# aleju/cat-generator

Measured on AMD Instinct MI355X. Metric: images/sec per G+D step, G32up-c 32x32 RGB bs=128 per GPU, higher is better.
Workload: dtype f32

## Files before the change

cat-generator_amd/csrc/common.h:

```cpp
#pragma once
#include <hip/hip_runtime.h>
#include <algorithm>
#include <stdint.h>
#include <stdio.h>
#include <string.h>
#include "../../include/catgan.h"

namespace cg {

char* err_buf();
int fail(const char* fmt, ...);

inline hipStream_t S(void* s) { return reinterpret_cast<hipStream_t>(s); }

#define CG_HIP(call)                                                              \
    do {                                                                          \
        hipError_t e__ = (call);                                                  \
        if (e__ != hipSuccess)                                                    \
            return cg::fail("%s:%d %s -> %s", __FILE__, __LINE__, #call,          \
                            hipGetErrorString(e__));                              \
    } while (0)

#define CG_LAUNCH_CHECK()                                                         \
    do {                                                                          \
        hipError_t e__ = hipGetLastError();                                       \
        if (e__ != hipSuccess)                                                    \
            return cg::fail("%s:%d kernel launch -> %s", __FILE__, __LINE__,      \
                            hipGetErrorString(e__));                              \
    } while (0)

#define CG_REQUIRE(cond, ...)                                                     \
    do {                                                                          \
        if (!(cond)) return cg::fail(__VA_ARGS__);                                \
    } while (0)

constexpr int kNumCU = 256;

#ifndef CG_TIMING_PROBE
#define CG_TIMING_PROBE 0
#endif
#define CG_PROBE_HALF(fam, T) (((CG_TIMING_PROBE) & (fam)) ? ((T) + 1) / 2 : (T))
constexpr int kEwWgsPerCU = 4, kColReduceWgsPerCU = 1;

enum Opt {
    OPT_SKINNY, OPT_GEMM_BK32, OPT_WINO_BK, OPT_NN_TILE, OPT_TN_TILE, OPT_NN_SPLITS, OPT_TN_SPLITS,
    OPT_XCD_SWIZZLE, OPT_NN_GLDS, OPT_TN_GLDS, OPT_WINO_GLDS, OPT_PAD_SKIP, OPT_WINO3, OPT_WINO_DGRAD_FUSE, OPT_WINO_DGRAD_FUSE_LAUNCHES,
    OPT_WINO3_LAUNCHES, OPT_PACK_WIDE, OPT_SAMPLER_ATOMIC_LAUNCHES, OPT_COUNT
};
long opt(Opt o);
void opt_count(Opt o);

static inline int cdiv(long a, long b) { return (int)((a + b - 1) / b); }

constexpr size_t kColScratchBytes = 8u << 20;
void* col_scratch(hipStream_t stream);
hipStream_t queue_stream(hipStream_t ref, int cls, int slot);
int queue_class(hipStream_t ref, hipStream_t s);

constexpr int MAXG = 4;
constexpr int kMaxStridedGroups = 36;
template <typename T>
__device__ __forceinline__ T sel4(int i, T a, T b, T c, T d) { return i == 0 ? a : (i == 1 ? b : (i == 2 ? c : d)); }
__device__ __forceinline__ float4 ld4(const float* p) { return *reinterpret_cast<const float4*>(p); }
__device__ __forceinline__ float f4c(const float4& v, int i) { return i == 0 ? v.x : (i == 1 ? v.y : (i == 2 ? v.z : v.w)); }
template <typename T>
static inline void set4(T& p0, T& p1, T& p2, T& p3, const T* src, int n) {
    T* const dst[MAXG] = {&p0, &p1, &p2, &p3};
    for (int i = 0; i < MAXG; ++i) *dst[i] = (src && i < n) ? src[i] : nullptr;
}
__device__ __host__ __forceinline__ int phase_map(int a, int d, int pad) { return ((a + d - pad) >> 1) - ((a - pad) >> 1); }
static inline int phase_kp(int k, int pad) { return phase_map(0, k - 1, pad) + 1; }

struct WgradParts {
    const float* part;
    const float* bias_part;
    float* const* gw;
    float* const* gb;
    long gws;
    int ngroups, S, Cin, Cout, kH, kW, pad, ups;
    float scale;
};
int wgrad_finish(hipStream_t st, const WgradParts& w, bool defer);
void wgrad_discard_all();

constexpr int kSkinnyWgradBlocks = 512;
bool skinny_ok(int ngroups, int Cin, int Cout, int kH, int kW, int padH, int padW, int ups);
size_t skinny_wgrad_ws_bytes(int Cin, int Cout);
void skinny_valu_forward(hipStream_t st, const float* x, const float* w, const float* bias, float* y, int N, int H, int W, int Cin, int Cout);
void skinny_valu_wgrad(hipStream_t st, const float* x, const float* dy, float* part, float* bias_part, int N, int H, int W, int Cin, int Cout,
                       int blocks, long ppb);
bool skinny_mfma_ok(int Cin, int Cout, int H, int W);
int skinny_mfma_forward(hipStream_t st, const float* x, const float* w, const float* bias, float* y, int N, int H, int W, int Cin, int Cout);
int skinny_mfma_wgrad(hipStream_t st, const float* x, const float* dy, float* part, float* bias_part, int N, int H, int W, int Cin, int Cout,
                      int max_blocks);

bool head_wgrad_ok(int N, int T, int C, int Co);
int head_wgrad(hipStream_t st, const float* x, const float* dy, float* gw, float* gb, int N, int T, int C, int Co, float scale);
constexpr int kWino3UOffset = 9 * 64 * 64, kWino3UFloats = 16 * 64 * 64;
static inline bool wino3_layer(int Cout, int Cin, int kH, int kW) { return Cout == 64 && Cin == 64 && kH == 3 && kW == 3; }
bool wino3_geom_ok(int ngroups, int N, int H, int W, int Cin, int Cout, int kH, int kW, int padH, int padW, int ups);
int wino3_note_pack(hipStream_t st, int n, const float* const* w, float* const* wf, float* const* wb, const int* Cout, const int* Cin,
                    const int* kH, const int* kW, const int* wb_map);
int wino3_forward(hipStream_t st, int ngroups, const float* const* x, const float* const* wpk, const float* const* bias, float* const* y,
                  int N, int H, int W);

static inline int ew_grid(long n, int per_block = 256) {
    long b = (n + per_block - 1) / per_block;
    if (b < 1) b = 1;
    const long cap = (long)kNumCU * kEwWgsPerCU;
    if (b > cap) b = cap;
    return (int)b;
}

static inline bool al16(const void* p) { return ((uintptr_t)p & 15) == 0; }
template <class... P>
static inline bool vec_ok(long n, const P*... p) { return n % 4 == 0 && (al16(p) && ...); }
// ... 247 lines not shown
```

cat-generator_amd/csrc/gemm.hip:

```cpp
#include "common.h"
#include <stdlib.h>
#include <algorithm>
#include <type_traits>

using cg::f4c;
using cg::kMaxStridedGroups;
using cg::ld4;
using cg::MAXG;
using cg::phase_kp;
using cg::sel4;
using cg::set4;

namespace {

typedef float f32x16 __attribute__((ext_vector_type(16)));
typedef unsigned int u32x4 __attribute__((ext_vector_type(4)));

constexpr int BK = 16;
constexpr unsigned OOB = 0x80000000u;
#ifdef CG_TRACE
__device__ unsigned long long* g_trace;
#define CG_STAMP(slot)                                                                                                  \
    do {                                                                                                                \
        if (threadIdx.x == 0 && g_trace) {                                                                              \
// ... 1735 lines not shown
}

int cg_conv2d_dgrad_ups2(void* stream, const float* dy, const float* wb_ph, float* dx_lo, int N, int Hp, int Wp, int Cin,
                         int Cout, int k, int pad, void* ws, size_t ws_bytes) {
    CG_REQUIRE(dy && wb_ph && dx_lo, "cg_conv2d_dgrad_ups2: null pointer");
    Geom g;
    if (check_dims(N, Hp, Wp, Cin, Cout, k, k, pad, pad, 1)) return 1;
    if (geom_phase_dgrad(g, N, Hp, Wp, Cin, Cout, k, pad)) return 1;
    return run_nn(cg::S(stream), g, 1, &dy, &wb_ph, nullptr, &dx_lo, ws, ws_bytes, "cg_conv2d_dgrad_ups2");
}

static size_t wgrad_ws_bytes_groups(int ngroups, int maxg, int N, int Hp, int Wp, int Cin, int Cout, int kH, int kW, int padH, int padW, int ups) {
    Geom g;
    if (ngroups < 1 || ngroups > maxg || conv_geom(g, N, Hp, Wp, Cin, Cout, kH, kW, padH, padW, ups)) return 0;
    const size_t reg = tn_ws_bytes(g, plan_tn(g, ngroups), ngroups);
    return cg::skinny_ok(ngroups, Cin, Cout, kH, kW, padH, padW, ups) ? std::max(reg, cg::skinny_wgrad_ws_bytes(Cin, Cout)) : reg;
}
size_t cg_conv2d_wgrad_workspace_bytes_grouped(int ngroups, int N, int Hp, int Wp, int Cin, int Cout, int kH, int kW,
                                               int padH, int padW, int ups) {
    return wgrad_ws_bytes_groups(ngroups, MAXG, N, Hp, Wp, Cin, Cout, kH, kW, padH, padW, ups);
}
size_t cg_conv2d_wgrad_workspace_bytes_strided(int ngroups, int N, int Hp, int Wp, int Cin, int Cout, int kH, int kW,
                                               int padH, int padW, int ups) {
    return wgrad_ws_bytes_groups(ngroups, kMaxStridedGroups, N, Hp, Wp, Cin, Cout, kH, kW, padH, padW, ups);
}
size_t cg_conv2d_wgrad_workspace_bytes(int N, int Hp, int Wp, int Cin, int Cout, int kH, int kW, int padH, int padW,
                                       int ups) {
    return cg_conv2d_wgrad_workspace_bytes_grouped(1, N, Hp, Wp, Cin, Cout, kH, kW, padH, padW, ups);
}

namespace {
int wgrad_impl(void* stream, int ngroups, const float* const* x, const float* const* dy, float* const* gw, float* const* gb, int N,
               int Hp, int Wp, int Cin, int Cout, int kH, int kW, int padH, int padW, int ups, float scale, void* ws, size_t ws_bytes,
               bool defer, long xgs = 0, long dgs = 0, long gws = 0, bool gemm_only = false);
}

int cg_conv2d_wgrad_grouped(void* stream, int ngroups, const float* const* x, const float* const* dy, float* const* gw,
                            float* const* gb, int N, int Hp, int Wp, int Cin, int Cout, int kH, int kW, int padH, int padW,
                            int ups, float scale, void* ws, size_t ws_bytes) {
    return wgrad_impl(stream, ngroups, x, dy, gw, gb, N, Hp, Wp, Cin, Cout, kH, kW, padH, padW, ups, scale, ws, ws_bytes, false);
}

int cg_conv2d_wgrad_grouped_deferred(void* stream, int ngroups, const float* const* x, const float* const* dy, float* const* gw,
                                     float* const* gb, int N, int Hp, int Wp, int Cin, int Cout, int kH, int kW, int padH, int padW,
                                     int ups, float scale, void* ws, size_t ws_bytes) {
    return wgrad_impl(stream, ngroups, x, dy, gw, gb, N, Hp, Wp, Cin, Cout, kH, kW, padH, padW, ups, scale, ws, ws_bytes, true);
}

int cg_conv2d_wgrad_strided(void* stream, int ngroups, const float* x, long x_stride, const float* dy, long dy_stride, float* gw,
                            long gw_stride, int N, int Hp, int Wp, int Cin, int Cout, int kH, int kW, int padH, int padW, int ups,
                            float scale, void* ws, size_t ws_bytes) {
    CG_REQUIRE(x && dy && gw && x_stride > 0 && dy_stride > 0 && gw_stride > 0, "cg_conv2d_wgrad_strided: bad arguments");
    CG_REQUIRE(ngroups >= 1 && ngroups <= kMaxStridedGroups, "cg_conv2d_wgrad_strided: 1..%d groups per launch", kMaxStridedGroups);
    return wgrad_impl(stream, ngroups, &x, &dy, &gw, nullptr, N, Hp, Wp, Cin, Cout, kH, kW, padH, padW, ups, scale, ws, ws_bytes, false,
                      x_stride, dy_stride, gw_stride);
}

int cg_conv2d_wgrad_gemm(void* stream, const float* x, const float* dy, int N, int Hp, int Wp, int Cin, int Cout, int kH, int kW, int padH,
                         int padW, int ups, void* ws, size_t ws_bytes) {
    CG_REQUIRE(x && dy && ws, "cg_conv2d_wgrad_gemm: null pointer");
    CG_REQUIRE(!cg::skinny_ok(1, Cin, Cout, kH, kW, padH, padW, ups), "cg_conv2d_wgrad_gemm: this geometry runs the skinny kernel, not the GEMM");
    float* gw = (float*)ws;
    return wgrad_impl(stream, 1, &x, &dy, &gw, nullptr, N, Hp, Wp, Cin, Cout, kH, kW, padH, padW, ups, 1.f, ws, ws_bytes, false, 0, 0, 0, true);
}

namespace {
void launch_tn_tile(const TNArgs& a, const TileCfg& tc, bool tng, dim3 grid, hipStream_t st, bool veca, bool vecb) {
    if (tng) {
        if (tc.bm == 128 && tc.bn == 128) launch_tng<128, 128, 2, 2>(a, grid, st);
        else if (tc.bm == 64 && tc.bn == 128) launch_tng<64, 128, 2, 2>(a, grid, st);
        else if (tc.bm == 128 && tc.bn == 64) launch_tng<128, 64, 2, 2>(a, grid, st);
        else if (tc.bm == 64 && tc.bn == 64) launch_tng<64, 64, 2, 2>(a, grid, st);
        else launch_tng<128, 32, 4, 1>(a, grid, st);
    }
    else if (tc.bm == 128 && tc.bn == 128) launch_tn<128, 128, 2, 2>(a, grid, st, veca, vecb);
    else if (tc.bm == 64 && tc.bn == 128) launch_tn<64, 128, 2, 2>(a, grid, st, veca, vecb);
    else if (tc.bm == 128 && tc.bn == 64) launch_tn<128, 64, 2, 2>(a, grid, st, veca, vecb);
    else if (tc.bm == 64 && tc.bn == 64) launch_tn<64, 64, 2, 2>(a, grid, st, veca, vecb);
    else launch_tn<128, 32, 4, 1>(a, grid, st, veca, vecb);
}

int wgrad_impl(void* stream, int ngroups, const float* const* x, const float* const* dy, float* const* gw, float* const* gb, int N,
               int Hp, int Wp, int Cin, int Cout, int kH, int kW, int padH, int padW, int ups, float scale, void* ws, size_t ws_bytes,
               bool defer, long xgs, long dgs, long gws_, bool gemm_only) {
    CG_REQUIRE(x && dy && gw, "cg_conv2d_wgrad: null pointer");
    const bool strided = xgs != 0;
    CG_REQUIRE(ngroups >= 1 && ngroups <= (strided ? kMaxStridedGroups : MAXG), "cg_conv2d_wgrad: 1..%d groups per launch", strided ? kMaxStridedGroups : MAXG);
    CG_REQUIRE(!strided || (!gb && !defer), "cg_conv2d_wgrad: strided groups carry no bias gradient and are not deferred");
    TNArgs a;
    memset(&a, 0, sizeof(a));
    if (conv_geom(a.g, N, Hp, Wp, Cin, Cout, kH, kW, padH, padW, ups)) return 1;
    const Geom& g = a.g;
    if (!strided && cg::skinny_ok(ngroups, Cin, Cout, kH, kW, padH, padW, ups) && x[0] && dy[0] && gw[0] && (uintptr_t)x[0] % 16 == 0 && ws &&
        ws_bytes >= cg::skinny_wgrad_ws_bytes(Cin, Cout) && (long)N * Hp * Wp < 0x7fffffffL) {
        hipStream_t st = cg::S(stream);
        const long npix = (long)N * Hp * Wp;
        const long ppb = (npix + cg::kSkinnyWgradBlocks - 1) / cg::kSkinnyWgradBlocks;
        int blocks = (int)((npix + ppb - 1) / ppb);
        float* part = (float*)ws;
        float* bpart = part + (size_t)cg::kSkinnyWgradBlocks * 9 * Cin * Cout;
        float* gb0 = gb ? gb[0] : nullptr;
        if (cg::opt(cg::OPT_SKINNY) == 1 && cg::skinny_mfma_ok(Cin, Cout, Hp, Wp)) {
            blocks = cg::skinny_mfma_wgrad(st, x[0], dy[0], part, gb0 ? bpart : nullptr, N, Hp, Wp, Cin, Cout, cg::kSkinnyWgradBlocks / 2);
            if (blocks < 0) return 1;
        }
        else cg::skinny_valu_wgrad(st, x[0], dy[0], part, gb0 ? bpart : nullptr, N, Hp, Wp, Cin, Cout, blocks, ppb);
        CG_LAUNCH_CHECK();
        const cg::WgradParts parts{part, gb0 ? bpart : nullptr, gw, gb, 0, 1, blocks, Cin, Cout, 3, 3, 1, 0, scale};
        return cg::wgrad_finish(st, parts, defer);
    }
    if (!strided && !gemm_only && ngroups == 1 && !ups && kH == Hp && kW == Wp && padH == 0 && padW == 0 && cg::opt(cg::OPT_PAD_SKIP) > 0 &&
        cg::opt(cg::OPT_TN_GLDS) && cg::head_wgrad_ok(N, kH * kW, Cin, Cout) && x[0] && dy[0] && gw[0] && (uintptr_t)x[0] % 16 == 0 &&
        (uintptr_t)dy[0] % 16 == 0 && (uintptr_t)gw[0] % 4 == 0)
        return cg::head_wgrad(cg::S(stream), x[0], dy[0], gw[0], gb ? gb[0] : nullptr, N, kH * kW, Cin, Cout, scale) != 0;
    TNPlan p = plan_tn(g, ngroups);
    const size_t need = tn_ws_bytes(g, p, ngroups);
    CG_REQUIRE(ws && ws_bytes >= need, "cg_conv2d_wgrad: workspace too small (%zu < %zu)", ws_bytes, need);
    const int nptr = strided ? 1 : ngroups;
    bool veca = Cin % 4 == 0, vecb = Cout % 4 == 0, any_gb = false;
    for (int i = 0; i < nptr; ++i) {
        CG_REQUIRE(x[i] && dy[i] && gw[i], "cg_conv2d_wgrad: null pointer (group %d)", i);
        veca = veca && ((uintptr_t)x[i] % 16 == 0);
        vecb = vecb && ((uintptr_t)dy[i] % 16 == 0);
        any_gb = any_gb || (gb && gb[i]);
    }
    if (strided) { veca = veca && xgs % 4 == 0; vecb = vecb && dgs % 4 == 0; }
    if (p.pm && !(veca && vecb)) p = plan_tn(g, ngroups, false);
    a.xgs = xgs; a.dgs = dgs;
    set4(a.x0, a.x1, a.x2, a.x3, x, nptr);
    set4(a.d0, a.d1, a.d2, a.d3, dy, nptr);
    a.ngroups = ngroups; a.part = (float*)ws; a.pchunk = p.pchunk;
    a.xcd_swizzle = (int)cg::opt(cg::OPT_XCD_SWIZZLE);
    const int ZP = ngroups * g.nphase;
    const long wplane = (long)g.Ktot * g.Cout;
    a.bias_part = any_gb ? (float*)ws + (size_t)p.splits * ZP * wplane : nullptr;
    hipStream_t st = cg::S(stream);
    dim3 grid(cg::cdiv(g.Ktot, p.tc.bm) * cg::cdiv(g.Cout, p.tc.bn), p.splits, ZP);
    if (p.pm && veca && vecb) a.pm_n = g.M / (g.Hg * g.Wg);
    launch_tn_tile(a, p.tc, a.pm_n || tng_ok(g, p.pchunk, veca, vecb), grid, st, veca, vecb);
    CG_LAUNCH_CHECK();
    if (gemm_only) return 0;
    const cg::WgradParts parts{(const float*)ws, a.bias_part, gw, gb, strided ? gws_ : 0, ngroups, p.splits, Cin, Cout, kH, kW, padH, ups, scale};
    return cg::wgrad_finish(st, parts, defer);
}

}

int cg_conv2d_wgrad(void* stream, const float* x, const float* dy, float* gw, float* gb, int N, int Hp, int Wp, int Cin,
                    int Cout, int kH, int kW, int padH, int padW, int ups, float scale, void* ws, size_t ws_bytes) {
    CG_REQUIRE(x && dy && gw, "cg_conv2d_wgrad: null pointer");
    return cg_conv2d_wgrad_grouped(stream, 1, &x, &dy, &gw, &gb, N, Hp, Wp, Cin, Cout, kH, kW, padH, padW, ups, scale, ws,
                                   ws_bytes);
}

}
```

cat-generator_amd/csrc/ops.hip:

```cpp
#include "common.h"
#include <stdarg.h>
#include <stdlib.h>
#include <algorithm>

namespace cg {
char* err_buf() {
    static thread_local char buf[512] = {0};
    return buf;
}
int fail(const char* fmt, ...) {
    va_list ap;
    va_start(ap, fmt);
    vsnprintf(err_buf(), 512, fmt, ap);
    va_end(ap);
    return 1;
}

namespace {
struct OptDef { const char* name; long dflt; };
const OptDef kOptDefs[OPT_COUNT] = {
    {"CG_SKINNY", 1}, {"CG_GEMM_BK32", 1}, {"CG_WINO_BK", 0}, {"CG_NN_TILE", 0}, {"CG_TN_TILE", 0}, {"CG_NN_SPLITS", 0}, {"CG_TN_SPLITS", 0},
    {"CG_XCD_SWIZZLE", 7}, {"CG_NN_GLDS", 1}, {"CG_TN_GLDS", 1}, {"CG_WINO_GLDS", 1}, {"CG_PAD_SKIP", 20}, {"CG_WINO3", 1},
    {"CG_WINO_DGRAD_FUSE", 1}, {"CG_WINO_DGRAD_FUSE_LAUNCHES", 0}, {"CG_WINO3_LAUNCHES", 0}, {"CG_PACK_WIDE", 1},
    {"CG_SAMPLER_ATOMIC_LAUNCHES", 0},
};
long g_opt_val[OPT_COUNT];
int g_opt_state[OPT_COUNT];
}

}
#include <chrono>
#include <mutex>
#include <unordered_map>
#include <vector>
namespace cg {
void* col_scratch(hipStream_t stream) {
    constexpr int kPool = 8, kReserve = 4;
    static std::unordered_map<hipStream_t, void*> blocks;
    static std::vector<void*> pool;
    static std::mutex mu;
    std::lock_guard<std::mutex> lk(mu);
    auto it = blocks.find(stream);
    if (it != blocks.end()) return it->second;
    hipStreamCaptureStatus st = hipStreamCaptureStatusNone;
    const bool capturing = stream && hipStreamIsCapturing(stream, &st) == hipSuccess && st != hipStreamCaptureStatusNone;
    if (capturing && pool.empty()) {
        cg::fail("column reduce: no scratch block left for a stream first used inside a graph capture (run one pass on it before cg_graph_begin)");
        return nullptr;
    }
    if (!capturing && (int)pool.size() <= kReserve) {
        char* p = nullptr;
        hipStreamCaptureMode mode = hipStreamCaptureModeRelaxed;
        (void)hipThreadExchangeStreamCaptureMode(&mode);
        const bool ok = hipMalloc((void**)&p, kColScratchBytes * kPool) == hipSuccess &&
                        hipMemsetAsync(p, 0, kColScratchBytes * kPool, stream) == hipSuccess &&
                        hipStreamSynchronize(stream) == hipSuccess;
        (void)hipThreadExchangeStreamCaptureMode(&mode);
// ... 1875 lines not shown
```

cat-generator_amd/csrc/wgrad_finish.hip:

```cpp
#include "common.h"
#include <mutex>
#include <unordered_map>
#include <vector>

namespace {

using cg::f4c;
using cg::ld4;
using cg::phase_map;
using cg::sel4;

template <bool UPS, int STEP>
__device__ __forceinline__ float fold(const float* pg, int tap, int ci, int co, int Cin, int Cout, int k, int pad, int kp, long plane, int S,
                                      long sstride, int sp0) {
    float s = 0.f;
    if (UPS) {
        const int dy = tap / k, dx = tap - dy * k;
        for (int sp = sp0; sp < S; sp += STEP)
#pragma unroll
            for (int p = 0; p < 4; ++p) {
                const int tp = phase_map(p >> 1, dy, pad) * kp + phase_map(p & 1, dx, pad);
                s += pg[(long)sp * sstride + (long)p * plane + ((long)tp * Cin + ci) * Cout + co];
            }
    } else {
        const long o = ((long)tap * Cin + ci) * Cout + co;
        constexpr int kInFlight = STEP == 8 ? 4 : 1;
#pragma unroll kInFlight
        for (int sp = sp0; sp < S; sp += STEP) s += pg[(long)sp * sstride + o];
    }
    return s;
}

__device__ __forceinline__ void add4(float4& s, const float4& p) { s.x += p.x; s.y += p.y; s.z += p.z; s.w += p.w; }
template <int STEP>
__device__ __forceinline__ float4 fold4(const float* src, int S, long sstride, int sp0) {
    float4 s = make_float4(0.f, 0.f, 0.f, 0.f);
    int sp = sp0;
    for (; sp + 3 * STEP < S; sp += 4 * STEP) {
        const float4 p0 = ld4(src + (long)sp * sstride), p1 = ld4(src + (long)(sp + STEP) * sstride);
        const float4 p2 = ld4(src + (long)(sp + 2 * STEP) * sstride), p3 = ld4(src + (long)(sp + 3 * STEP) * sstride);
        add4(s, p0); add4(s, p1); add4(s, p2); add4(s, p3);
    }
    for (; sp < S; sp += STEP) add4(s, ld4(src + (long)sp * sstride));
    return s;
}

__device__ __forceinline__ float lane_groups_sum(float (*sh)[33], int ol) {
    float t = 0.f;
#pragma unroll
    for (int r = 0; r < 8; ++r) t += sh[r][ol];
    return t;
}

__device__ __forceinline__ void bias_sum_block(float (*sh)[33], const float* bp, float* gb, int c0, int S, int P, long bsstride, int Cout, float scale) {
    const int cl = threadIdx.x & 31, ln = threadIdx.x >> 5;
    const int c = c0 + cl;
    float s = 0.f;
    if (c < Cout)
        for (int i = ln; i < S * P; i += 8) s += bp[(long)(i / P) * bsstride + (long)(i % P) * Cout + c];
    sh[ln][cl] = s;
    __syncthreads();
    if (ln == 0 && c < Cout) gb[c] += scale * lane_groups_sum(sh, cl);
}

template <bool UPS>
__global__ __launch_bounds__(256) void wgrad_reduce_kernel(const float* part, float* gw, int Cin, int Cout, int k, int KK,
                                                           int pad, int kp, int S, float scale, int CI_T, long sstride) {
    extern __shared__ float sh[];
    const int ci0 = blockIdx.x * CI_T, co0 = blockIdx.y * 32;
    const long plane = (long)(UPS ? kp * kp : KK) * Cin * Cout;
    const int n1 = KK * CI_T * 32;
    for (int idx = threadIdx.x; idx < n1; idx += 256) {
        const int co_l = idx & 31;
        const int r = idx >> 5;
        const int ci_l = r % CI_T, tap = r / CI_T;
        const int ci = ci0 + ci_l, co = co0 + co_l;
        float s = 0.f;
        if (ci < Cin && co < Cout) s = fold<UPS, 1>(part, tap, ci, co, Cin, Cout, k, pad, kp, plane, S, sstride, 0);
        sh[(ci_l * KK + tap) * 33 + co_l] = s;
    }
    __syncthreads();
    const int run = CI_T * KK;
    for (int idx = threadIdx.x; idx < n1; idx += 256) {
        const int j = idx % run, co_l = idx / run;
        const int ci_l = j / KK, tap = j - ci_l * KK;
        const int ci = ci0 + ci_l, co = co0 + co_l;
        if (ci < Cin && co < Cout) {
            float* dst = gw + ((long)co * Cin + ci) * KK + tap;
            *dst += scale * sh[j * 33 + co_l];
        }
    }
}

__global__ __launch_bounds__(256) void bias_part_reduce_kernel(const float* bp, float* gb, int S, int P, long sstride, int Cout, float scale) {
    __shared__ float sh[8][33];
    bias_sum_block(sh, bp, gb, blockIdx.x * 32, S, P, sstride, Cout, scale);
}

struct RedPtrs { float* gw0; float* gw1; float* gw2; float* gw3; float* gb0; float* gb1; float* gb2; float* gb3;
                 long gws; };
struct RedJob {
    const float* part; const float* bias_part;
    RedPtrs rp;
    long sstride, gstride, bsstride;
    int Cin, Cout, k, KK, pad, kp, S, P, ups, ngroups, wblocks, bblocks;
    int block0;
    float scale;
    int tr;
    int v4;
};
constexpr int kRedJobs = 20;
struct RedJobTable { RedJob j[kRedJobs]; int n; };

__device__ __forceinline__ float* gw_of(const RedPtrs& rp, int group) {
    return rp.gws ? rp.gw0 + (long)group * rp.gws : sel4(group, rp.gw0, rp.gw1, rp.gw2, rp.gw3);
}

template <bool UPS>
__device__ __forceinline__ void wgrad_reduce_small(float (*sh)[33], const RedJob& J, int group, int bx) {
    const int ol = threadIdx.x & 31, ln = threadIdx.x >> 5;
    const long total = (long)J.KK * J.Cin * J.Cout, plane = (long)(UPS ? J.kp * J.kp : J.KK) * J.Cin * J.Cout;
    const long i = bx * 32L + ol;
    int co = 0, ci = 0, tap = 0;
    float s = 0.f;
// ... 109 lines not shown
    } else if (!w.ups && w.Cout % 4 == 0 && cg::al16(w.part) && job.sstride % 4 == 0 && job.gstride % 4 == 0) {
        job.v4 = 1; job.wblocks = cg::cdiv(relems, 128);
    }
    return job;
}

int small_reduce(hipStream_t st, bool defer, const RedJob& job) {
    if (defer) {
        std::lock_guard<std::mutex> lk(g_red_mu);
        g_red_queue[st].push_back(job);
        return 0;
    }
    hipLaunchKernelGGL(wgrad_reduce_small_kernel, dim3(job.wblocks + job.bblocks, job.ngroups), dim3(256), 0, st, job);
    CG_LAUNCH_CHECK();
    return 0;
}

}

int cg::wgrad_finish(hipStream_t st, const WgradParts& w, bool defer) {
    const RedJob job = red_job(w, defer);
    const int Cin = w.Cin, Cout = w.Cout, KK = job.KK;
    if (w.gws && transposable(w) && !w.bias_part) {
        hipLaunchKernelGGL(wgrad_reduce_t_kernel, dim3(Cin / 32, Cout / 32, w.ngroups), dim3(256), 0, st, w.part, w.gw[0], w.gws, Cin, Cout, w.S,
                           job.sstride, job.gstride, w.scale);
        CG_LAUNCH_CHECK();
        return 0;
    }
    int ci_t = KK == 1 ? 64 : 8;
    while (ci_t > 1 && (size_t)KK * ci_t * 33 * sizeof(float) > 60000) ci_t >>= 1;
    const size_t shb = (size_t)KK * ci_t * 33 * sizeof(float);
    const dim3 rgrid(cg::cdiv(Cin, ci_t), cg::cdiv(Cout, 32));
    if ((long)rgrid.x * rgrid.y < cg::kNumCU) return small_reduce(st, defer, job);
    for (int gi = 0; gi < w.ngroups; ++gi) {
        const float* pg = w.part + gi * job.gstride;
        float* gwi = w.gws ? w.gw[0] + gi * w.gws : w.gw[gi];
        hipLaunchKernelGGL(w.ups ? wgrad_reduce_kernel<true> : wgrad_reduce_kernel<false>, rgrid, dim3(256), shb, st, pg, gwi, Cin, Cout, w.kH, KK,
                           w.pad, job.kp, w.S, w.scale, ci_t, job.sstride);
        CG_LAUNCH_CHECK();
        if (w.gb && w.gb[gi]) {
            hipLaunchKernelGGL(bias_part_reduce_kernel, dim3(cg::cdiv(Cout, 32)), dim3(256), 0, st, w.bias_part + (long)gi * job.P * Cout, w.gb[gi],
                               w.S, job.P, job.bsstride, Cout, w.scale);
            CG_LAUNCH_CHECK();
        }
    }
    return 0;
}

void cg::wgrad_discard_all() {
    std::lock_guard<std::mutex> lk(g_red_mu);
    for (auto& kv : g_red_queue) kv.second.clear();
}

extern "C" {

int cg_conv2d_wgrad_pending(void* stream, int* njobs) {
    CG_REQUIRE(njobs, "cg_conv2d_wgrad_pending: null pointer");
    std::lock_guard<std::mutex> lk(g_red_mu);
    auto it = g_red_queue.find(cg::S(stream));
    *njobs = it == g_red_queue.end() ? 0 : (int)it->second.size();
    return 0;
}

int cg_conv2d_wgrad_flush(void* stream) {
    hipStream_t st = cg::S(stream);
    std::vector<RedJob> jobs;
    {
        std::lock_guard<std::mutex> lk(g_red_mu);
        auto it = g_red_queue.find(st);
        if (it == g_red_queue.end() || it->second.empty()) return 0;
        jobs.swap(it->second);
// ... 19 lines not shown
```

cat-generator_amd/csrc/winograd.hip:

```cpp
#include "common.h"
#include <algorithm>
#include <type_traits>
#include <stdlib.h>

namespace {

typedef float f32x16 __attribute__((ext_vector_type(16)));

using cg::ld4;
__device__ __forceinline__ void st4(float* p, float4 v) { *reinterpret_cast<float4*>(p) = v; }
using cg::f4c;
__device__ __forceinline__ float4 f4add(float4 a, float4 b) { return make_float4(a.x + b.x, a.y + b.y, a.z + b.z, a.w + b.w); }
__device__ __forceinline__ float4 f4sub(float4 a, float4 b) { return make_float4(a.x - b.x, a.y - b.y, a.z - b.z, a.w - b.w); }
__device__ __forceinline__ float4 f4neg(float4 a) { return make_float4(-a.x, -a.y, -a.z, -a.w); }

template <class Body>
__device__ __forceinline__ void wino_tile_walk(int N, int Hl, int Wl, int C, Body body) {
    const int cq_n = C >> 2;
    const int tH = Hl >> 1, tW = Wl >> 1;
    const long T = (long)N * tH * tW;
    const long total = T * cq_n;
    for (long idx = blockIdx.x * 256L + threadIdx.x; idx < total; idx += gridDim.x * 256L) {
        const int cq = (int)(idx % cq_n);
        const long tile = idx / cq_n;
// ... 727 lines not shown
    for (int row = 0; row < 4; ++row) {
        if (xy == row) {
#pragma unroll
            for (int o = 0; o < 4; ++o) {
                if (cyr[o >> 1] == 0.f) continue;
#pragma unroll
                for (int ni = 0; ni < 2; ++ni) {
                    f32x16 Y;
                    add_row(o, ni, Y);
                    if (row == 3) store_out(o, ni, Y);
                    else {
                        float* Xo = X + (o * 2 + ni) * 1024;
#pragma unroll
                        for (int r = 0; r < 16; ++r) Xo[r * 64 + lane] = Y[r];
                    }
                }
            }
        } else if (row == 3 && xy < 2) {
#pragma unroll
            for (int ni = 0; ni < 2; ++ni) {
                f32x16 Y;
                const float* Xo = X + (xy * 2 + ni) * 1024;
#pragma unroll
                for (int r = 0; r < 16; ++r) Y[r] = Xo[r * 64 + lane];
                if (xy == 0) store_out(0, ni, Y); else store_out(1, ni, Y);
            }
        }
        if (row < 3) __syncthreads();
    }
}

__device__ __host__ __forceinline__ int wino_phase_map(int a, int d) { return ((a + d - 2) >> 1) - ((a - 2) >> 1); }

__global__ __launch_bounds__(256) void wino_wgrad_finish_kernel(const float* __restrict__ dUt, float* __restrict__ gw, int Cout,
                                                                int Cin, float scale) {
    const long total = (long)Cout * Cin;
    const long xs = 4L * Cout * Cin;
    for (long idx = blockIdx.x * 256L + threadIdx.x; idx < total; idx += gridDim.x * 256L) {
        const int ci = (int)(idx % Cin);
        const int co = (int)(idx / Cin);
        float acc[25];
#pragma unroll
        for (int t = 0; t < 25; ++t) acc[t] = 0.f;
#pragma unroll
        for (int p = 0; p < 4; ++p) {
            float u[4][4];
#pragma unroll
            for (int xi = 0; xi < 16; ++xi) u[xi >> 2][xi & 3] = dUt[xi * xs + ((long)p * Cout + co) * Cin + ci];
            float t[3][4];
#pragma unroll
            for (int c = 0; c < 4; ++c) {
                t[0][c] = u[0][c] + 0.5f * (u[1][c] + u[2][c]);
                t[1][c] = 0.5f * (u[1][c] - u[2][c]);
                t[2][c] = 0.5f * (u[1][c] + u[2][c]) + u[3][c];
            }
            float g[3][3];
#pragma unroll
            for (int r = 0; r < 3; ++r) {
                g[r][0] = t[r][0] + 0.5f * (t[r][1] + t[r][2]);
                g[r][1] = 0.5f * (t[r][1] - t[r][2]);
                g[r][2] = 0.5f * (t[r][1] + t[r][2]) + t[r][3];
            }
#pragma unroll
            for (int dy = 0; dy < 5; ++dy)
#pragma unroll
                for (int dx = 0; dx < 5; ++dx) acc[dy * 5 + dx] += g[wino_phase_map(p >> 1, dy)][wino_phase_map(p & 1, dx)];
        }
        float* dst = gw + idx * 25;
#pragma unroll
        for (int t = 0; t < 25; ++t) dst[t] += scale * acc[t];
    }
}

bool wino_dims_ok(int N, int Hp, int Wp, int Cin, int Cout) {
    return N > 0 && Hp > 0 && Wp > 0 && (Hp & 1) == 0 && (Wp & 1) == 0 && Cin > 0 && Cout > 0 && Cin % 128 == 0 &&
           Cout % 128 == 0  && (long)N * Hp * Wp * std::max(Cin, 4 * Cout) * 4L < (1L << 40);
}

bool glds_ok(long T, int K, int Nc) {
    return cg::opt(cg::OPT_WINO_GLDS) != 0 && T * K * 4L < 0x7fffffffL && 16L * K * Nc * 4L < 0x7fffffffL;
}

int wino_gemm_launch(void* stream, const float* v, const float* u, const float* bias, float* y, int N, int Hp, int Wp,
                     int Cin, int Cout, int dgrad, float* stats, int npos, int kslices) {
    CG_REQUIRE(v && u && y, "cg_conv2d_ups2_wino_gemm: null pointer");
    CG_REQUIRE(wino_dims_ok(N, Hp, Wp, Cin, Cout), "cg_conv2d_ups2_wino_gemm: unsupported dimensions");
    const int T = N * (Hp / 2) * (Wp / 2);
    WinoArgs a;
    a.V = v; a.U = u; a.bias = bias; a.y = y; a.T = T; a.tH = Hp / 2; a.tW = Wp / 2; a.stats = stats;
    a.xcd = (int)cg::opt(cg::OPT_XCD_SWIZZLE);
    a.vpp = npos == 9 && !dgrad ? 1 : 0;
    a.kz = 0;
    a.lg_tw = a.lg_th = -1;
    CG_REQUIRE(!stats || !dgrad, "wino_gemm: statistics only on the forward launch");
    if (dgrad) { a.K = 4 * Cout; a.Nc = Cin; a.so = 1; a.Ho = Hp; a.Wo = Wp; }
    else { a.K = Cin; a.Nc = Cout; a.so = 2; a.Ho = 2 * Hp; a.Wo = 2 * Wp; }
    const int bk = (int)cg::opt(cg::OPT_WINO_BK);
    CG_REQUIRE(kslices <= 1 || (dgrad && a.K % kslices == 0 && (a.K / kslices) % 64 == 0), "wino_gemm: K slices only on the data gradient, in multiples of 64 rows");
    if (kslices > 1) a.kz = a.K / kslices;
    {
        auto lg = [](int v) { int l = 0; while ((1 << l) < v) ++l; return (1 << l) == v ? l : -1; };
        const long ybytes = (long)N * a.Ho * a.Wo * a.Nc * 4L;
        if (lg(a.tW) >= 0 && lg(a.tH) >= 0 && ybytes < 0x7fffffffL) { a.lg_tw = lg(a.tW); a.lg_th = lg(a.tH); }
// ... 190 lines not shown
int cg_conv2d_ups2_wino_dgrad_split(void* stream, const float* dy, const float* u_bwd, float* dx_lo, float* v_dy, float* part, int N, int Hp,
                                    int Wp, int Cin, int Cout) {
    const int sl = wino_dgrad_slices(N, Hp, Wp, Cin, Cout);
    if (sl <= 1 || !part) return cg_conv2d_ups2_wino_dgrad(stream, dy, u_bwd, dx_lo, v_dy, N, Hp, Wp, Cin, Cout);
    CG_REQUIRE(dy && u_bwd && dx_lo && v_dy, "cg_conv2d_ups2_wino_dgrad_split: null pointer");
    return wino_dgrad_pair(stream, dy, u_bwd, dx_lo, v_dy, part, N, Hp, Wp, Cin, Cout, 16, sl);
}

size_t cg_conv2d_ups2_wino_wgrad_workspace_bytes(int N, int Hp, int Wp, int Cin, int Cout) {
    if (!wino_dims_ok(N, Hp, Wp, Cin, Cout)) return 0;
    const size_t T = (size_t)N * (Hp / 2) * (Wp / 2);
    return wino_align(16 * T * 4 * Cout * sizeof(float)) + wino_align((size_t)16 * 4 * Cout * Cin * sizeof(float)) + wino_bias_ws_bytes(Cout) +
           cg_conv2d_wgrad_workspace_bytes_strided(16, (int)T, 1, 1, Cin, 4 * Cout, 1, 1, 0, 0, 0);
}

int cg_conv2d_ups2_wino_wgrad(void* stream, const float* v, const float* dy, float* gw_canonical, float* gb, int N, int Hp,
                              int Wp, int Cin, int Cout, float scale, void* ws, size_t ws_bytes) {
    CG_REQUIRE(v && dy && gw_canonical, "cg_conv2d_ups2_wino_wgrad: null pointer");
    CG_REQUIRE(wino_dims_ok(N, Hp, Wp, Cin, Cout), "cg_conv2d_ups2_wino_wgrad: unsupported dimensions");
    const size_t need = cg_conv2d_ups2_wino_wgrad_workspace_bytes(N, Hp, Wp, Cin, Cout);
    CG_REQUIRE(ws && ws_bytes >= need && (uintptr_t)ws % 16 == 0, "cg_conv2d_ups2_wino_wgrad: workspace too small (%zu < %zu)",
               ws_bytes, need);
    hipStream_t st = cg::S(stream);
    const int T = N * (Hp / 2) * (Wp / 2);
    const int C4 = 4 * Cout;
    char* base = (char*)ws;
    float* mdy = (float*)base;                    base += wino_align((size_t)16 * T * C4 * sizeof(float));
    float* dut = (float*)base;                    base += wino_align((size_t)16 * C4 * Cin * sizeof(float));
    void* bws = base;                             base += wino_bias_ws_bytes(Cout);
    void* tws = base;
    const size_t tws_bytes = ws_bytes - (size_t)(base - (char*)ws);
    hipLaunchKernelGGL(wino_dy_transform_kernel, dim3(cg::ew_grid((long)T * Cout)), dim3(256), 0, st, dy, mdy, N, Hp, Wp, Cout);
    CG_LAUNCH_CHECK();
    CG_HIP(hipMemsetAsync(dut, 0, (size_t)16 * C4 * Cin * sizeof(float), st));
    if (cg_conv2d_wgrad_strided(stream, 16, v, (long)T * Cin, mdy, (long)T * C4, dut, (long)C4 * Cin, T, 1, 1, Cin, C4, 1, 1, 0, 0, 0, 1.f,
                                tws, tws_bytes)) return 1;
    hipLaunchKernelGGL(wino_wgrad_finish_kernel, dim3(cg::ew_grid((long)Cout * Cin)), dim3(256), 0, st, dut, gw_canonical, Cout,
                       Cin, scale);
    CG_LAUNCH_CHECK();
    if (gb) return cg_bias_grad(stream, dy, gb, (long)N * 4 * Hp * Wp, Cout, scale, bws, wino_align(sizeof(double) * Cout));
    return 0;
}

}
```

Before: 23610.

## Fuse wgrad split-K reduction with phase/Winograd fold into single-pass kernels

```diff
diff --git a/cat-generator_amd/csrc/common.h b/cat-generator_amd/csrc/common.h
--- a/cat-generator_amd/csrc/common.h
+++ b/cat-generator_amd/csrc/common.h
@@ -45,7 +45,7 @@
 enum Opt {
     OPT_SKINNY, OPT_GEMM_BK32, OPT_WINO_BK, OPT_NN_TILE, OPT_TN_TILE, OPT_NN_SPLITS, OPT_TN_SPLITS,
     OPT_XCD_SWIZZLE, OPT_NN_GLDS, OPT_TN_GLDS, OPT_WINO_GLDS, OPT_PAD_SKIP, OPT_WINO3, OPT_WINO_DGRAD_FUSE, OPT_WINO_DGRAD_FUSE_LAUNCHES,
-    OPT_WINO3_LAUNCHES, OPT_PACK_WIDE, OPT_SAMPLER_ATOMIC_LAUNCHES, OPT_COUNT
+    OPT_WINO3_LAUNCHES, OPT_PACK_WIDE, OPT_SAMPLER_ATOMIC_LAUNCHES, OPT_WGRAD_STREAM, OPT_COUNT
 };
 long opt(Opt o);
 void opt_count(Opt o);
@@ -82,6 +82,8 @@
 };
 int wgrad_finish(hipStream_t st, const WgradParts& w, bool defer);
 void wgrad_discard_all();
+int wgrad_strided_partials(hipStream_t st, int ngroups, const float* x, long x_stride, const float* dy, long dy_stride, int M, int Cin, int Cout,
+                           void* ws, size_t ws_bytes, int* splits);
 
 constexpr int kSkinnyWgradBlocks = 512;
 bool skinny_ok(int ngroups, int Cin, int Cout, int kH, int kW, int padH, int padW, int ups);
diff --git a/cat-generator_amd/csrc/gemm.hip b/cat-generator_amd/csrc/gemm.hip
--- a/cat-generator_amd/csrc/gemm.hip
+++ b/cat-generator_amd/csrc/gemm.hip
@@ -1791,7 +1791,7 @@
 namespace {
 int wgrad_impl(void* stream, int ngroups, const float* const* x, const float* const* dy, float* const* gw, float* const* gb, int N,
                int Hp, int Wp, int Cin, int Cout, int kH, int kW, int padH, int padW, int ups, float scale, void* ws, size_t ws_bytes,
-               bool defer, long xgs = 0, long dgs = 0, long gws = 0, bool gemm_only = false);
+               bool defer, long xgs = 0, long dgs = 0, long gws = 0, bool gemm_only = false, int* splits_out = nullptr);
 }
 
 int cg_conv2d_wgrad_grouped(void* stream, int ngroups, const float* const* x, const float* const* dy, float* const* gw,
@@ -1841,7 +1841,7 @@
 
 int wgrad_impl(void* stream, int ngroups, const float* const* x, const float* const* dy, float* const* gw, float* const* gb, int N,
                int Hp, int Wp, int Cin, int Cout, int kH, int kW, int padH, int padW, int ups, float scale, void* ws, size_t ws_bytes,
-               bool defer, long xgs, long dgs, long gws_, bool gemm_only) {
+               bool defer, long xgs, long dgs, long gws_, bool gemm_only, int* splits_out) {
     CG_REQUIRE(x && dy && gw, "cg_conv2d_wgrad: null pointer");
     const bool strided = xgs != 0;
     CG_REQUIRE(ngroups >= 1 && ngroups <= (strided ? kMaxStridedGroups : MAXG), "cg_conv2d_wgrad: 1..%d groups per launch", strided ? kMaxStridedGroups : MAXG);
@@ -1898,6 +1898,7 @@
     if (p.pm && veca && vecb) a.pm_n = g.M / (g.Hg * g.Wg);
     launch_tn_tile(a, p.tc, a.pm_n || tng_ok(g, p.pchunk, veca, vecb), grid, st, veca, vecb);
     CG_LAUNCH_CHECK();
+    if (splits_out) *splits_out = p.splits;
     if (gemm_only) return 0;
     const cg::WgradParts parts{(const float*)ws, a.bias_part, gw, gb, strided ? gws_ : 0, ngroups, p.splits, Cin, Cout, kH, kW, padH, ups, scale};
     return cg::wgrad_finish(st, parts, defer);
@@ -1913,3 +1914,11 @@
 }
 
 }
+
+int cg::wgrad_strided_partials(hipStream_t st, int ngroups, const float* x, long x_stride, const float* dy, long dy_stride, int M, int Cin,
+                               int Cout, void* ws, size_t ws_bytes, int* splits) {
+    CG_REQUIRE(x && dy && ws && splits && x_stride > 0 && dy_stride > 0, "wgrad_strided_partials: bad arguments");
+    float* gw = (float*)ws;
+    return wgrad_impl((void*)st, ngroups, &x, &dy, &gw, nullptr, M, 1, 1, Cin, Cout, 1, 1, 0, 0, 0, 1.f, ws, ws_bytes, false, x_stride, dy_stride,
+                      0, true, splits);
+}
diff --git a/cat-generator_amd/csrc/ops.hip b/cat-generator_amd/csrc/ops.hip
--- a/cat-generator_amd/csrc/ops.hip
+++ b/cat-generator_amd/csrc/ops.hip
@@ -22,7 +22,7 @@
     {"CG_SKINNY", 1}, {"CG_GEMM_BK32", 1}, {"CG_WINO_BK", 0}, {"CG_NN_TILE", 0}, {"CG_TN_TILE", 0}, {"CG_NN_SPLITS", 0}, {"CG_TN_SPLITS", 0},
     {"CG_XCD_SWIZZLE", 7}, {"CG_NN_GLDS", 1}, {"CG_TN_GLDS", 1}, {"CG_WINO_GLDS", 1}, {"CG_PAD_SKIP", 20}, {"CG_WINO3", 1},
     {"CG_WINO_DGRAD_FUSE", 1}, {"CG_WINO_DGRAD_FUSE_LAUNCHES", 0}, {"CG_WINO3_LAUNCHES", 0}, {"CG_PACK_WIDE", 1},
-    {"CG_SAMPLER_ATOMIC_LAUNCHES", 0},
+    {"CG_SAMPLER_ATOMIC_LAUNCHES", 0}, {"CG_WGRAD_STREAM", 1},
 };
 long g_opt_val[OPT_COUNT];
 int g_opt_state[OPT_COUNT];
diff --git a/cat-generator_amd/csrc/wgrad_finish.hip b/cat-generator_amd/csrc/wgrad_finish.hip
--- a/cat-generator_amd/csrc/wgrad_finish.hip
+++ b/cat-generator_amd/csrc/wgrad_finish.hip
@@ -1,5 +1,6 @@
 #include "common.h"
 #include <mutex>
+#include <type_traits>
 #include <unordered_map>
 #include <vector>
 
@@ -9,6 +10,8 @@
 using cg::ld4;
 using cg::phase_map;
 using cg::sel4;
+
+__device__ __forceinline__ int phase_tap(int p, int dy, int dx, int pad, int kp) { return phase_map(p >> 1, dy, pad) * kp + phase_map(p & 1, dx, pad); }
 
 template <bool UPS, int STEP>
 __device__ __forceinline__ float fold(const float* pg, int tap, int ci, int co, int Cin, int Cout, int k, int pad, int kp, long plane, int S,
@@ -19,7 +22,7 @@
         for (int sp = sp0; sp < S; sp += STEP)
 #pragma unroll
             for (int p = 0; p < 4; ++p) {
-                const int tp = phase_map(p >> 1, dy, pad) * kp + phase_map(p & 1, dx, pad);
+                const int tp = phase_tap(p, dy, dx, pad, kp);
                 s += pg[(long)sp * sstride + (long)p * plane + ((long)tp * Cin + ci) * Cout + co];
             }
     } else {
@@ -61,6 +64,28 @@
     sh[ln][cl] = s;
     __syncthreads();
     if (ln == 0 && c < Cout) gb[c] += scale * lane_groups_sum(sh, cl);
+}
+
+
+template <int B>
+__device__ __forceinline__ void tile_accumulate(const float* sh, float* gw, int ci0, int co0, int Cin, int Cout, int KK, int CI_T, float scale) {
+    const int run = CI_T * KK, n1 = run * 32, nt = blockDim.x;
+    for (int idx0 = threadIdx.x; idx0 < n1; idx0 += B * nt) {
+        float* dst[B];
+        float old[B], s[B];
+#pragma unroll
+        for (int b = 0; b < B; ++b) {
+            const int idx = idx0 + b * nt;
+            const int j = idx % run, co_l = idx / run;
+            const int ci_l = j / KK, tap = j - ci_l * KK;
+            const int ci = ci0 + ci_l, co = co0 + co_l;
+            dst[b] = idx < n1 && ci < Cin && co < Cout ? gw + ((long)co * Cin + ci) * KK + tap : nullptr;
+            if (dst[b]) { old[b] = *dst[b]; s[b] = sh[j * 33 + co_l]; }
+        }
+#pragma unroll
+        for (int b = 0; b < B; ++b)
+            if (dst[b]) *dst[b] = old[b] + scale * s[b];
+    }
 }
 
 template <bool UPS>
@@ -80,16 +105,49 @@
         sh[(ci_l * KK + tap) * 33 + co_l] = s;
     }
     __syncthreads();
-    const int run = CI_T * KK;
-    for (int idx = threadIdx.x; idx < n1; idx += 256) {
-        const int j = idx % run, co_l = idx / run;
-        const int ci_l = j / KK, tap = j - ci_l * KK;
-        const int ci = ci0 + ci_l, co = co0 + co_l;
-        if (ci < Cin && co < Cout) {
-            float* dst = gw + ((long)co * Cin + ci) * KK + tap;
-            *dst += scale * sh[j * 33 + co_l];
-        }
-    }
+    tile_accumulate<1>(sh, gw, ci0, co0, Cin, Cout, KK, CI_T, scale);
+}
+
+template <int K>
+__global__ __launch_bounds__(256) void wgrad_reduce_ups_once_kernel(const float* __restrict__ part, float* __restrict__ gw, int Cin, int Cout,
+                                                                    int S, float scale, long sstride) {
+    constexpr int PAD = K / 2, KP = (K + 1) / 2, KK = K * K, CI_T = 8;
+    __shared__ float sh[CI_T * KK * 33];
+    const int co0 = blockIdx.x * 32, ci0 = blockIdx.y * CI_T;
+    const int ci_l = threadIdx.x >> 5, co_l = threadIdx.x & 31;
+    const int ci = ci0 + ci_l, co = co0 + co_l;
+    float acc[KK];
+#pragma unroll
+    for (int t = 0; t < KK; ++t) acc[t] = 0.f;
+    if (ci < Cin && co < Cout) {
+        const long tstride = (long)Cin * Cout;
+        const float* src = part + (long)ci * Cout + co;
+        auto splits = [&](auto uc) {
+            constexpr int U = decltype(uc)::value, NV = 4 * KP * KP;
+            float v[U][NV];
+#pragma unroll
+            for (int u = 0; u < U; ++u)
+#pragma unroll
+                for (int i = 0; i < NV; ++i) v[u][i] = src[u * sstride + i * tstride];
+#pragma unroll
+            for (int u = 0; u < U; ++u)
+#pragma unroll
+                for (int p = 0; p < 4; ++p)
+#pragma unroll
+                    for (int dy = 0; dy < K; ++dy)
+#pragma unroll
+                        for (int dx = 0; dx < K; ++dx) acc[dy * K + dx] += v[u][p * KP * KP + phase_tap(p, dy, dx, PAD, KP)];
+            src += U * sstride;
+        };
+        constexpr int kAhead = K == 3 ? 2 : 1;
+        int sp = 0;
+        for (; sp + kAhead <= S; sp += kAhead) splits(std::integral_constant<int, kAhead>{});
+        for (; sp < S; ++sp) splits(std::integral_constant<int, 1>{});
+    }
+#pragma unroll
+    for (int t = 0; t < KK; ++t) sh[(ci_l * KK + t) * 33 + co_l] = acc[t];
+    __syncthreads();
+    tile_accumulate<K == 3 ? 9 : 5>(sh, gw, ci0, co0, Cin, Cout, KK, CI_T, scale);
 }
 
 __global__ __launch_bounds__(256) void bias_part_reduce_kernel(const float* bp, float* gb, int S, int P, long sstride, int Cout, float scale) {
@@ -265,11 +323,16 @@
     const size_t shb = (size_t)KK * ci_t * 33 * sizeof(float);
     const dim3 rgrid(cg::cdiv(Cin, ci_t), cg::cdiv(Cout, 32));
     if ((long)rgrid.x * rgrid.y < cg::kNumCU) return small_reduce(st, defer, job);
+    const bool once = w.ups && cg::opt(cg::OPT_WGRAD_STREAM) != 0 && (w.kH == 3 || w.kH == 5) && w.kW == w.kH && w.pad == w.kH / 2 && ci_t == 8;
     for (int gi = 0; gi < w.ngroups; ++gi) {
         const float* pg = w.part + gi * job.gstride;
         float* gwi = w.gws ? w.gw[0] + gi * w.gws : w.gw[gi];
-        hipLaunchKernelGGL(w.ups ? wgrad_reduce_kernel<true> : wgrad_reduce_kernel<false>, rgrid, dim3(256), shb, st, pg, gwi, Cin, Cout, w.kH, KK,
-                           w.pad, job.kp, w.S, w.scale, ci_t, job.sstride);
+        if (once)
+            hipLaunchKernelGGL(w.kH == 3 ? wgrad_reduce_ups_once_kernel<3> : wgrad_reduce_ups_once_kernel<5>, dim3(rgrid.y, rgrid.x), dim3(256), 0, st,
+                               pg, gwi, Cin, Cout, w.S, w.scale, job.sstride);
+        else
+            hipLaunchKernelGGL(w.ups ? wgrad_reduce_kernel<true> : wgrad_reduce_kernel<false>, rgrid, dim3(256), shb, st, pg, gwi, Cin, Cout, w.kH, KK,
+                               w.pad, job.kp, w.S, w.scale, ci_t, job.sstride);
         CG_LAUNCH_CHECK();
         if (w.gb && w.gb[gi]) {
             hipLaunchKernelGGL(bias_part_reduce_kernel, dim3(cg::cdiv(Cout, 32)), dim3(256), 0, st, w.bias_part + (long)gi * job.P * Cout, w.gb[gi],
diff --git a/cat-generator_amd/csrc/winograd.hip b/cat-generator_amd/csrc/winograd.hip
--- a/cat-generator_amd/csrc/winograd.hip
+++ b/cat-generator_amd/csrc/winograd.hip
@@ -783,6 +783,30 @@
 
 __device__ __host__ __forceinline__ int wino_phase_map(int a, int d) { return ((a + d - 2) >> 1) - ((a - 2) >> 1); }
 
+__device__ __forceinline__ void wino_gt_u_g(const float (&u)[4][4], float (&g)[3][3]) {
+    float t[3][4];
+#pragma unroll
+    for (int c = 0; c < 4; ++c) {
+        t[0][c] = u[0][c] + 0.5f * (u[1][c] + u[2][c]);
+        t[1][c] = 0.5f * (u[1][c] - u[2][c]);
+        t[2][c] = 0.5f * (u[1][c] + u[2][c]) + u[3][c];
+    }
+#pragma unroll
+    for (int r = 0; r < 3; ++r) {
+        g[r][0] = t[r][0] + 0.5f * (t[r][1] + t[r][2]);
+        g[r][1] = 0.5f * (t[r][1] - t[r][2]);
+        g[r][2] = 0.5f * (t[r][1] + t[r][2]) + t[r][3];
+    }
+}
+template <class G>
+__device__ __forceinline__ void wino_phase_scatter(float (&acc)[25], int p, G g) {
+#pragma unroll
+    for (int dy = 0; dy < 5; ++dy)
+#pragma unroll
+        for (int dx = 0; dx < 5; ++dx) acc[dy * 5 + dx] += g(wino_phase_map(p >> 1, dy), wino_phase_map(p & 1, dx));
+}
+__device__ __forceinline__ float wino_gw_sum(float old, float scale, float v) { return old + scale * v; }
+
 __global__ __launch_bounds__(256) void wino_wgrad_finish_kernel(const float* __restrict__ dUt, float* __restrict__ gw, int Cout,
                                                                 int Cin, float scale) {
     const long total = (long)Cout * Cin;
@@ -798,28 +822,86 @@
             float u[4][4];
 #pragma unroll
             for (int xi = 0; xi < 16; ++xi) u[xi >> 2][xi & 3] = dUt[xi * xs + ((long)p * Cout + co) * Cin + ci];
-            float t[3][4];
-#pragma unroll
-            for (int c = 0; c < 4; ++c) {
-                t[0][c] = u[0][c] + 0.5f * (u[1][c] + u[2][c]);
-                t[1][c] = 0.5f * (u[1][c] - u[2][c]);
-                t[2][c] = 0.5f * (u[1][c] + u[2][c]) + u[3][c];
-            }
             float g[3][3];
-#pragma unroll
-            for (int r = 0; r < 3; ++r) {
-                g[r][0] = t[r][0] + 0.5f * (t[r][1] + t[r][2]);
-                g[r][1] = 0.5f * (t[r][1] - t[r][2]);
-                g[r][2] = 0.5f * (t[r][1] + t[r][2]) + t[r][3];
-            }
-#pragma unroll
-            for (int dy = 0; dy < 5; ++dy)
-#pragma unroll
-                for (int dx = 0; dx < 5; ++dx) acc[dy * 5 + dx] += g[wino_phase_map(p >> 1, dy)][wino_phase_map(p & 1, dx)];
+            wino_gt_u_g(u, g);
+            wino_phase_scatter(acc, p, [&](int r, int c) { return g[r][c]; });
         }
         float* dst = gw + idx * 25;
 #pragma unroll
-        for (int t = 0; t < 25; ++t) dst[t] += scale * acc[t];
+        for (int t = 0; t < 25; ++t) dst[t] = wino_gw_sum(dst[t], scale, acc[t]);
+    }
+}
+
+constexpr int kTailCi = 4, kTailThreads = 4 * kTailCi * 8;
+constexpr int kTailGs = kTailCi * 9 + 1, kTailOs = kTailCi * 25 + 1;
+__global__ __launch_bounds__(kTailThreads) void wino_wgrad_tail_kernel(const float* __restrict__ part, float* __restrict__ gw, int Cout, int Cin,
+                                                                       int S, long sstride, float scale) {
+    __shared__ float sg[4 * 32 * kTailGs];
+    __shared__ float so[32 * kTailOs];
+    const int ci0 = blockIdx.x * kTailCi, co0 = blockIdx.y * 32;
+    const int tid = threadIdx.x;
+    {
+        const int cq = tid & 7, ci_l = (tid >> 3) % kTailCi, p = tid / (8 * kTailCi);
+        const long C4 = 4L * Cout, xs = C4 * Cin;
+        const float* src = part + (long)(ci0 + ci_l) * C4 + (long)p * Cout + co0 + 4 * cq;
+        float4 u4[16];
+#pragma unroll
+        for (int xi = 0; xi < 16; ++xi) u4[xi] = make_float4(0.f, 0.f, 0.f, 0.f);
+        auto splits = [&](auto uc) {
+            constexpr int U = decltype(uc)::value;
+            float4 v[U][16];
+#pragma unroll
+            for (int k = 0; k < U; ++k)
+#pragma unroll
+                for (int xi = 0; xi < 16; ++xi) v[k][xi] = ld4(src + k * sstride + xi * xs);
+#pragma unroll
+            for (int k = 0; k < U; ++k)
+#pragma unroll
+                for (int xi = 0; xi < 16; ++xi) u4[xi] = f4add(u4[xi], v[k][xi]);
+            src += U * sstride;
+        };
+        int sp = 0;
+        for (; sp + 2 <= S; sp += 2) splits(std::integral_constant<int, 2>{});
+        for (; sp < S; ++sp) splits(std::integral_constant<int, 1>{});
+#pragma unroll
+        for (int j = 0; j < 4; ++j) {
+            float u[4][4], g[3][3];
+#pragma unroll
+            for (int xi = 0; xi < 16; ++xi) u[xi >> 2][xi & 3] = f4c(u4[xi], j);
+            wino_gt_u_g(u, g);
+            float* dst = sg + (p * 32 + 4 * cq + j) * kTailGs + ci_l * 9;
+#pragma unroll
+            for (int r = 0; r < 9; ++r) dst[r] = g[r / 3][r % 3];
+        }
+    }
+    __syncthreads();
+    {
+        const int ci_l = tid % kTailCi, co_l = tid / kTailCi;
+        float acc[25];
+#pragma unroll
+        for (int t = 0; t < 25; ++t) acc[t] = 0.f;
+#pragma unroll
+        for (int p = 0; p < 4; ++p) {
+            const float* g = sg + (p * 32 + co_l) * kTailGs + ci_l * 9;
+            wino_phase_scatter(acc, p, [&](int r, int c) { return g[r * 3 + c]; });
+        }
+#pragma unroll
+        for (int t = 0; t < 25; ++t) so[co_l * kTailOs + ci_l * 25 + t] = acc[t];
+    }
+    __syncthreads();
+    constexpr int run = kTailCi * 25, per = 32 * run / kTailThreads;
+    float* dst[per];
+    float old[per];
+#pragma unroll
+    for (int b = 0; b < per; ++b) {
+        const int idx = tid + b * kTailThreads, co_l = idx / run, j = idx - co_l * run;
+        dst[b] = gw + ((long)(co0 + co_l) * Cin + ci0) * 25 + j;
+        old[b] = *dst[b];
+    }
+#pragma unroll
+    for (int b = 0; b < per; ++b) {
+        const int idx = tid + b * kTailThreads, co_l = idx / run, j = idx - co_l * run;
+        *dst[b] = wino_gw_sum(old[b], scale, so[co_l * kTailOs + j]);
     }
 }
 
@@ -1076,11 +1158,18 @@
     const size_t tws_bytes = ws_bytes - (size_t)(base - (char*)ws);
     hipLaunchKernelGGL(wino_dy_transform_kernel, dim3(cg::ew_grid((long)T * Cout)), dim3(256), 0, st, dy, mdy, N, Hp, Wp, Cout);
     CG_LAUNCH_CHECK();
-    CG_HIP(hipMemsetAsync(dut, 0, (size_t)16 * C4 * Cin * sizeof(float), st));
-    if (cg_conv2d_wgrad_strided(stream, 16, v, (long)T * Cin, mdy, (long)T * C4, dut, (long)C4 * Cin, T, 1, 1, Cin, C4, 1, 1, 0, 0, 0, 1.f,
-                                tws, tws_bytes)) return 1;
-    hipLaunchKernelGGL(wino_wgrad_finish_kernel, dim3(cg::ew_grid((long)Cout * Cin)), dim3(256), 0, st, dut, gw_canonical, Cout,
-                       Cin, scale);
+    if (cg::opt(cg::OPT_WGRAD_STREAM) != 0) {
+        int splits = 0;
+        if (cg::wgrad_strided_partials(st, 16, v, (long)T * Cin, mdy, (long)T * C4, T, Cin, C4, tws, tws_bytes, &splits)) return 1;
+        hipLaunchKernelGGL(wino_wgrad_tail_kernel, dim3(Cin / kTailCi, Cout / 32), dim3(kTailThreads), 0, st, (const float*)tws, gw_canonical, Cout,
+                           Cin, splits, 16L * Cin * C4, scale);
+    } else {
+        CG_HIP(hipMemsetAsync(dut, 0, (size_t)16 * C4 * Cin * sizeof(float), st));
+        if (cg_conv2d_wgrad_strided(stream, 16, v, (long)T * Cin, mdy, (long)T * C4, dut, (long)C4 * Cin, T, 1, 1, Cin, C4, 1, 1, 0, 0, 0, 1.f,
+                                    tws, tws_bytes)) return 1;
+        hipLaunchKernelGGL(wino_wgrad_finish_kernel, dim3(cg::ew_grid((long)Cout * Cin)), dim3(256), 0, st, dut, gw_canonical, Cout,
+                           Cin, scale);
+    }
     CG_LAUNCH_CHECK();
     if (gb) return cg_bias_grad(stream, dy, gb, (long)N * 4 * Hp * Wp, Cout, scale, bws, wino_align(sizeof(double) * Cout));
     return 0;
```

Result: no change. 23720 (median of 6 runs) (+0.4%).
